# Aikku93/ulc-codec

Hardware: AMD Instinct MI355X
Metric: encode+decode Msamples/s at BlockSize=2048 stereo (channel-samples through encode+decode, VBR -50, 32 blocks per stream per call) (higher is better)
Workload: dtype f32; 1 GPU; vbr50 (configs[1] encode, configs[2] decode): Batch=4096 independent 44.1 kHz stereo streams/GPU x 32 blocks, BlockSize=2048, VBR -50; step = encode then decode; config=vbr50, mode=both, streams_per_gpu=4096, block_size=2048, channels=2, parallelism=batch split over 1 GPU(s), no collective on the data path

## Files before the change

ulc-codec_amd/csrc/ulcx_enc.hip:

```cpp
#include "ulcx_enc_dev.h"

static size_t ulcx_enc_xf_lds_bytes(int BS, int C) {
    if (BS > 8192) return (size_t)BS * 4;
    int ps = ulcx_xf_pad_shift(BS, C);
    size_t z = (size_t)4 * (BS + (BS >> ps)) * 4;
    size_t full = z + (size_t)BS * 2 + 32 + (C > 2 ? (size_t)BS * 2 : 0);
    return full <= ULCX_LDS_LIMIT ? full : z + (size_t)BS * 2 + 32;
}

static size_t ulcx_enc_xfa_lds_bytes(int BS, int C) {
    if (BS > 8192) return (size_t)BS * 4;
    int ps = ulcx_xf_pad_shift(BS, C);
    return (size_t)2 * (BS + (BS >> ps)) * 4 + (size_t)BS * 2 + 32;
}

#define CK(x) do { hipError_t e_ = (x); if (e_ != hipSuccess) { ulcx_set_error("%s: %s", #x, hipGetErrorString(e_)); return ULCX_ERR_HIP; } } while (0)
#define TRY(x) do { int rc_ = (x); if (rc_) return rc_; } while (0)

typedef void (*RangeKernel)(UlcxEncCtx, int, int);
typedef void (*PassKernel)(UlcxEncCtx, int);
typedef void (*CallKernel)(UlcxEncCtx);

static RangeKernel wc_energy_fn(const UlcxEncCtx &c) { return c.pcm16 ? k_wc_energy<int16_t> : k_wc_energy<float>; }
static RangeKernel wc_ef_fn(const UlcxEncCtx &c) { return c.pcm16 ? k_wc_ef<EF_NW, int16_t> : k_wc_ef<EF_NW, float>; }
static CallKernel state_update_fn(const UlcxEncCtx &c) { return c.pcm16 ? k_state_update<int16_t> : k_state_update<float>; }

template <typename IN> static RangeKernel xf_fn_in(const UlcxEncCtx &c, bool mdctOnly) {
    if (c.BS > 8192) return mdctOnly ? k_xfa_big<IN> : k_xf_big<IN>;
    if (c.C == 2) return mdctOnly ? k_xfa<true, IN> : k_xf<true, IN>;
    return mdctOnly ? k_xfa<false, IN> : k_xf<false, IN>;
}
static RangeKernel xf_fn(const UlcxEncCtx &c, bool mdctOnly) { return c.pcm16 ? xf_fn_in<int16_t>(c, mdctOnly) : xf_fn_in<float>(c, mdctOnly); }

template <int PASS> static PassKernel select_fn_pass(const UlcxEncCtx &c, bool pair, bool rates) {
#define SEL(R, L) (rates ? (PassKernel)k_select_wave_rates<R, L, PASS> : (PassKernel)k_select_wave<R, L, PASS>)
    switch (c.C * c.BS / 64) {
        case 128:
            if (pair) return rates ? k_select_pair_rates<64, 12, PASS> : k_select_pair<64, 12, PASS>;
            return SEL(128, 0);
        case 64: return c.lgBS == 11 ? SEL(64, 11) : SEL(64, 0);
        case 32: return SEL(32, 0);
        case 16: return SEL(16, 0);
        case 8:  return SEL(8, 0);
        case 4:  return SEL(4, 0);
        default: return nullptr;
    }
#undef SEL
}
static PassKernel select_fn(const UlcxEncCtx &c, bool pair, bool rates, int pass) {
    return pass == 1 ? select_fn_pass<1>(c, pair, rates) : pass == 2 ? select_fn_pass<2>(c, pair, rates) : select_fn_pass<0>(c, pair, rates);
}

static int allow_lds(const void *fn, size_t lds) {
    if (lds > 48 * 1024) CK(hipFuncSetAttribute(fn, hipFuncAttributeMaxDynamicSharedMemorySize, (int)lds));
    return ULCX_OK;
}

static void launch_wc_energy(const UlcxEncCtx &c, unsigned grid, hipStream_t st, int k0, int k1) {
    hipLaunchKernelGGL(wc_energy_fn(c), dim3(grid), dim3(WG), 0, st, c, k0, k1);
}

static void launch_wc_ef(const UlcxEncCtx &c, hipStream_t st, int k0, int k1) {
    static_assert(EF_LDS_BYTES <= 48 * 1024, "k_wc_ef: raise the dynamic LDS limit with hipFuncSetAttribute");
    hipLaunchKernelGGL(wc_ef_fn(c), dim3((c.B + EF_SPW - 1) / EF_SPW), dim3(EF_NW * 64), EF_LDS_BYTES, st, c, k0, k1);
}

static void launch_state_update(const UlcxEncCtx &c, hipStream_t st) {
    hipLaunchKernelGGL(state_update_fn(c), dim3(c.B), dim3(WG), 0, st, c);
}

const char *const ulcx_enc_stage_names[ULCX_ENC_STAGES_REPORTED] = {
    "k_wc_energy", "k_wc_forward", "k_wc_backward", "k_wc_integrate", "k_wc_decide",
    "k_xf", "k_cplx", "k_pbark", "k_mask",
    "k_select", "k_nbark", "(k_nline: gone)", "k_heapsel", "k_nsums", "k_tails", "k_encode_wave", "k_encode_units", "k_pack", "cbr_probe_passes", "k_state_update", "wc_pipeline_exposed",
};

struct StageMarks { hipEvent_t *ev; int stage; };
#define MARK(mk, s) do { if ((mk).ev) CK(hipEventRecord((mk).ev[(mk).stage++], s)); } while (0)

enum { ULCX_FRONT_ENCODE = 0, ULCX_FRONT_ANALYSE = 1, ULCX_FRONT_ANALYSE_KXF = 2, ULCX_FRONT_WC_ONLY = 3 };
static int launch_front(const UlcxEncCtx &c, hipStream_t st, StageMarks &mk, const UlcxEncAux &aux, const int what) {
    UlcxEncSync &sy = aux.sync;
    hipStream_t side = sy.side, side2 = sy.side2, side3 = sy.side3;
    const int SG = (c.B + 63) / 64;
    const int nCh = aux.wcPipe;
    const bool mdctOnly = (what == ULCX_FRONT_ANALYSE);
    const RangeKernel xf = (what == ULCX_FRONT_WC_ONLY) ? nullptr : xf_fn(c, mdctOnly);
    const size_t lds = mdctOnly ? ulcx_enc_xfa_lds_bytes(c.BS, c.C) : ulcx_enc_xf_lds_bytes(c.BS, c.C);
    if (xf) TRY(allow_lds((const void *)xf, lds));
    auto transform = [&](int k0, int k1) {
        if (xf) hipLaunchKernelGGL(xf, dim3((unsigned)((c.B * (k1 - k0) + 7) / 8) * 8), dim3(WG), lds, st, c, k0, k1);
    };
    const bool wcFuse = c.C == 2 && aux.wcFuse;
    aux.nXf = 0;
    if (nCh <= 1) {
        if (wcFuse) { MARK(mk, st); launch_wc_ef(c, st, 0, c.K);                                                  MARK(mk, st); }
        else {
        launch_wc_energy(c, (unsigned)(SG * ((c.K * c.BS) / 64)), st, 0, c.K);                                    MARK(mk, st);
        hipLaunchKernelGGL(k_wc_forward, dim3((c.B * 2 + 63) / 64), dim3(64), 0, st, c, 0, c.K);                  MARK(mk, st);
        }
        hipLaunchKernelGGL(k_wc_backward, dim3(SG * c.K), dim3(64), 0, st, c, 0, c.K);                            MARK(mk, st);
        hipLaunchKernelGGL(k_wc_integrate, dim3((c.B + 63) / 64), dim3(64), 0, st, c, 0, c.K);                    MARK(mk, st);
        hipLaunchKernelGGL(k_wc_decide, dim3((c.B * c.K + 63) / 64), dim3(64), 0, st, c, 0, c.K);                 MARK(mk, st);
        transform(0, c.K);
        MARK(mk, st);
        return ULCX_OK;
    }
    for (int i = 0; i < 5; i++) MARK(mk, st);
    int nW = aux.wcSteps;
    if (nW < 0) nW = (c.K >= 8) ? 4 : 0;
    if (nW > ULCX_WC_MAXCH) nW = ULCX_WC_MAXCH;
    if (nW > c.K) nW = c.K;
    const bool sameCuts = nW < 1;
    if (sameCuts) nW = nCh;
    int cut[ULCX_XF_MAXCH + 1];
    cut[0] = 0; cut[1] = 1;
    for (int j = 2; j <= nCh; j++) cut[j] = 1 + (c.K - 1) * (j - 1) / (nCh - 1);
    int wcs[ULCX_WC_MAXCH + 1];
    for (int w = 0; w <= nW; w++) wcs[w] = sameCuts ? cut[w] : (int)((long long)c.K * w / nW);
    CK(hipEventRecord(sy.wcStart, st));
    CK(hipStreamWaitEvent(side, sy.wcStart, 0));
    int jx = 0;
    for (int w = 0; w < nW; w++) {
        const int k0 = wcs[w], k1 = wcs[w + 1], kc = k1 - k0;
        if (wcFuse) launch_wc_ef(c, side, k0, k1);
        else {
            launch_wc_energy(c, (unsigned)(SG * ((kc * c.BS) / 64)), side, k0, k1);
            hipLaunchKernelGGL(k_wc_forward, dim3((c.B * 2 + 63) / 64), dim3(64), 0, side, c, k0, k1);
        }
        CK(hipEventRecord(sy.wcForward[w], side));
        CK(hipStreamWaitEvent(side2, sy.wcForward[w], 0));
        hipLaunchKernelGGL(k_wc_backward, dim3(SG * kc), dim3(64), 0, side2, c, k0, k1);
        CK(hipEventRecord(sy.wcBackward[w], side2));
        CK(hipStreamWaitEvent(side3, sy.wcBackward[w], 0));
        hipLaunchKernelGGL(k_wc_integrate, dim3((c.B + 63) / 64), dim3(64), 0, side3, c, k0, k1);
        hipLaunchKernelGGL(k_wc_decide, dim3((c.B * kc + 63) / 64), dim3(64), 0, side3, c, k0, k1);
        CK(hipEventRecord(sy.wcDecided[w], side3));
        while (jx < nCh && cut[jx + 1] <= k1) {
            CK(hipStreamWaitEvent(st, sy.wcDecided[w], 0));
            if (mk.ev) CK(hipEventRecord(sy.xfTiming[2 * jx], st));
            if (!(ULCX_DBG(c) & 0x2000))
            transform(cut[jx], cut[jx + 1]);
            if (mk.ev) CK(hipEventRecord(sy.xfTiming[2 * jx + 1], st));
            CK(hipEventRecord(sy.xfChunkDone[jx], st));
            jx++;
        }
    }
    aux.nXf = nCh;
    MARK(mk, st);
    for (int j = 0; j < nCh; j++) {
        CK(hipStreamWaitEvent(side, sy.xfChunkDone[j], 0));
        const int kc2 = cut[j + 1] - cut[j];
        if (what == ULCX_FRONT_ENCODE) hipLaunchKernelGGL(k_cplx, dim3((c.B * kc2 + 63) / 64), dim3(64), 0, side, c, cut[j], cut[j + 1]);
        else hipLaunchKernelGGL(k_cplxa, dim3((c.B * kc2 + 63) / 64), dim3(64), 0, side, c, cut[j], cut[j + 1]);
    }
    CK(hipEventRecord(sy.cplxChunksDone, side));
    return ULCX_OK;
}

struct EncPlan {
    int NB, N, nUnits;
    bool aside;
    int probes;
    size_t barkLds;
    bool selWave, selPair;
    size_t selLds;
    int ldsEntries, fbGrid; size_t heapLds;
    WaveCaps capS, capM, capF;
    bool haveFull, haveMid;
    int nsSlots;
};
static int enc_probes(const UlcxEncCtx &c, int N) {
    int n = 0;
    if (c.mode != ULCX_MODE_VBR || c.rates != nullptr) { n = 2; for (int m = N; m > 1; m >>= 1) n++; }
    return n;
}
static EncPlan enc_plan(const UlcxEncCtx &c, const UlcxEncAux &aux) {
    EncPlan p;
    p.NB = c.B * c.K; p.N = c.C * c.BS; p.nUnits = p.NB * c.C * 4;
    p.aside = aux.sync.side != nullptr;
    p.probes = enc_probes(c, p.N);
    p.barkLds = (size_t)c.barkRing * 3 * 64 * 8 + (size_t)2 * BK_TILE_FLOATS * 4;
    const int R = p.N / 64;
    p.selWave = (R == 4 || R == 8 || R == 16 || R == 32 || R == 64 || R == 128);
    p.selPair = (R == 128 && c.C == 2 && c.selPair);
    p.selLds = (size_t)(p.selPair ? 1 : 4) * ulcx_sel_lds_words(c.BS) * sizeof(float);
    p.ldsEntries = ((size_t)p.N * 8 <= ULCX_HEAP_LDS_BYTES) ? p.N : 0;
    p.heapLds = p.ldsEntries ? (size_t)p.N * 8 + (size_t)p.N / 8 : 0;
    p.fbGrid = p.NB < ULCX_HEAP_GRID ? p.NB : ULCX_HEAP_GRID;
    p.capS = { WAVE_SK, WAVE_SZ, WAVE_SN };
    p.capF = { (c.BS + 63) & ~63, ((c.BS / 2) + 63) & ~63, 4 * c.BS + 64 };
    while ((size_t)wavecaps_lds(p.capF) * 4 > 150 * 1024) {
        p.capF.k = (p.capF.k / 2 + 63) & ~63; p.capF.z = (p.capF.z / 2 + 63) & ~63; p.capF.nyb = p.capF.nyb / 2 + 32;
    }
    p.haveFull = p.capF.k > p.capS.k;
    p.capM = { 1024, 512, 4096 };
    p.haveMid = p.capM.k < p.capF.k;
    p.nsSlots = aux.nsSlots;
    return p;
}

static void launch_noise(const UlcxEncCtx &c, const EncPlan &p, hipStream_t s2) {
    if (c.barkRing) {
        hipLaunchKernelGGL(k_bark_uniform<true>, dim3((p.NB * c.C + 63) / 64), dim3(256), p.barkLds, s2, c);
        hipLaunchKernelGGL(k_bark_levels<true>, dim3((unsigned)(((size_t)p.NB * c.C * 32 + WG - 1) / WG)), dim3(WG), 0, s2, c);
    }
    hipLaunchKernelGGL(k_nbark, dim3((p.nUnits + 63) / 64), dim3(64), 0, s2, c, c.barkRing ? 1 : 0);
}

static int launch_psy(const UlcxEncCtx &c, const EncPlan &p, UlcxEncSync &sy, hipStream_t st, StageMarks &mk, bool cplxChunked) {
    if (c.barkRing) { TRY(allow_lds((const void *)k_bark_uniform<true>, p.barkLds)); TRY(allow_lds((const void *)k_bark_uniform<false>, p.barkLds)); }
    if (p.aside) {
        CK(hipEventRecord(sy.noiseFork, st));
        CK(hipStreamWaitEvent(sy.side3, sy.noiseFork, 0));
        if (cplxChunked) CK(hipStreamWaitEvent(sy.side3, sy.cplxChunksDone, 0));
        else hipLaunchKernelGGL(k_cplx, dim3((p.NB + 63) / 64), dim3(64), 0, sy.side3, c, 0, c.K);
        CK(hipEventRecord(sy.cplxDone, sy.side3));
        MARK(mk, st);
        launch_state_update(c, sy.side3);
        CK(hipEventRecord(sy.stateDone, sy.side3));
        CK(hipStreamWaitEvent(sy.side2, sy.noiseFork, 0));
        launch_noise(c, p, sy.side2);
        CK(hipEventRecord(sy.noiseDone, sy.side2));
    } else { hipLaunchKernelGGL(k_cplx, dim3((p.NB + 63) / 64), dim3(64), 0, st, c, 0, c.K);                MARK(mk, st); }
    const bool uniP = c.barkRing != 0;
    if (uniP) {
        hipLaunchKernelGGL(k_bark_uniform<false>, dim3((p.NB + 63) / 64), dim3(256), p.barkLds, st, c);
        hipLaunchKernelGGL(k_bark_levels<false>, dim3((unsigned)(((size_t)p.NB * 32 + WG - 1) / WG)), dim3(WG), 0, st, c);
    }
    hipLaunchKernelGGL(k_pbark, dim3((p.NB * 4 + 63) / 64), dim3(64), 0, st, c, uniP ? 1 : 0);            MARK(mk, st);
    MARK(mk, st);
    if (p.aside) CK(hipStreamWaitEvent(st, sy.cplxDone, 0));
    return ULCX_OK;
}

static int launch_select_wave(const UlcxEncCtx &c, const EncPlan &p, hipStream_t st, bool rates, int pass, int fin) {
    const PassKernel fn = select_fn(c, p.selPair, rates, pass);
    TRY(allow_lds((const void *)fn, p.selLds));
    if (p.selPair) hipLaunchKernelGGL(fn, dim3(p.NB), dim3(128), p.selLds, st, c, fin);
    else hipLaunchKernelGGL(fn, dim3((p.NB + 3) / 4), dim3(256), p.selLds, st, c, fin);
    return ULCX_OK;
}
static int launch_select(const UlcxEncCtx &c, const EncPlan &p, hipStream_t st, int fin) {
    if (!p.selWave) { hipLaunchKernelGGL(k_select, dim3(p.NB), dim3(WG), 0, st, c, fin); return ULCX_OK; }
    const bool rates = c.rates && c.selPass;
    TRY(launch_select_wave(c, p, st, rates, c.selPass, fin));
    if (rates && fin) TRY(launch_select_wave(c, p, st, true, 0, fin));
    return ULCX_OK;
}

static int launch_encode(const UlcxEncCtx &cc, const EncPlan &p, UlcxEncSync &sy, hipStream_t s2, int fin, StageMarks &mk) {
    const bool fb2 = (cc.fbMode == 2);
    const int NB = p.NB, fbW = NB < 128 ? NB : 128;
    if (cc.useGapSums) {
        const size_t glds = nsums_lds_bytes(p.N, cc.C);
        TRY(allow_lds((const void *)k_nsums, glds));
        const bool tailAside = !fb2 && p.aside;
        const unsigned tg = (unsigned)((p.nUnits + TAILS_U - 1) / TAILS_U);
        if (tailAside) {
            CK(hipEventRecord(sy.tailFork, s2));
            CK(hipStreamWaitEvent(sy.side2, sy.tailFork, 0));
            hipLaunchKernelGGL(k_tails, dim3(tg), dim3(WG), 0, sy.side2, cc, fin);
            CK(hipEventRecord(sy.tailDone, sy.side2));
        }
        const int nsGrid = NB < p.nsSlots ? NB : p.nsSlots;
        hipLaunchKernelGGL(k_nsums, dim3(fb2 ? fbW : nsGrid), dim3(WG), glds, s2, cc, fin);
        MARK(mk, s2);
        if (tailAside) CK(hipStreamWaitEvent(s2, sy.tailDone, 0));
        else hipLaunchKernelGGL(k_tails, dim3(fb2 ? fbW : tg), dim3(WG), 0, s2, cc, fin);
        MARK(mk, s2);
    } else { MARK(mk, s2); MARK(mk, s2); }
    if (cc.useWave) {
        const int nBC = NB * cc.C;
        hipLaunchKernelGGL(k_encode_wave<true>, dim3(fb2 ? fbW : (nBC + 3) / 4), dim3(256), (size_t)wavecaps_lds(p.capS) * 4 + 16, s2, cc, fin, p.capS, p.haveFull ? 0 : 2);
        if (p.haveFull) {
            const WaveCaps capR = (p.haveMid && (fb2 || (p.probes > 0 && !fin))) ? p.capM : p.capF;
            hipLaunchKernelGGL(k_encode_wave<false>, dim3(fb2 ? fbW : ((nBC + 3) / 4 < 512 ? (nBC + 3) / 4 : 512)), dim3(256), (size_t)wavecaps_lds(capR) * 4 + 16, s2, cc, fin, capR, 1);
        }
    }
    MARK(mk, s2);
    hipLaunchKernelGGL(k_encode_units, dim3(fb2 ? fbW : (p.nUnits + 63) / 64), dim3(64), 0, s2, cc, fin);
    MARK(mk, s2);
    if (!fin && !fb2) hipLaunchKernelGGL(k_rate_step, dim3((NB + 255) / 256), dim3(256), 0, s2, cc);
    else hipLaunchKernelGGL(k_pack, dim3(fb2 ? (fbW + 3) / 4 : (NB + 3) / 4), dim3(256), 0, s2, cc, fin);
    MARK(mk, s2);
    return ULCX_OK;
}

static UlcxEncCtx exact_ctx(const UlcxEncCtx &c, int lo) { UlcxEncCtx cf = c; cf.fbMode = 2; cf.fbLo = lo; cf.fbHi = lo + c.rankSlots; return cf; }
static void exact_sort(const UlcxEncCtx &c, const EncPlan &p, hipStream_t s2, int lo) {
    const UlcxEncCtx cf = exact_ctx(c, lo);
    if (p.ldsEntries) hipLaunchKernelGGL(k_heapsel_pipe, dim3(p.fbGrid), dim3(64), p.heapLds, s2, cf, p.probes > 0 ? 1 : 0);
    else hipLaunchKernelGGL(k_heapsel, dim3(p.fbGrid), dim3(64), p.heapLds, s2, cf, p.ldsEntries);
}
static int exact_passes(const UlcxEncCtx &c, const EncPlan &p, UlcxEncSync &sy, hipStream_t s2, int lo) {
    const UlcxEncCtx cf = exact_ctx(c, lo);
    StageMarks none = { nullptr, 0 };
    for (int pass = 0; pass <= p.probes; pass++) {
        const int fin = (pass == p.probes) ? 1 : 0;
        const bool fromSort = (p.probes == 0 && p.ldsEntries);
        if (!fromSort) hipLaunchKernelGGL(k_keep_ranks, dim3(p.fbGrid), dim3(WG), 0, s2, cf, fin);
        if (cf.useWave && !(fromSort && lo == 0)) CK(hipMemsetAsync(cf.slow + p.NB + 1, 0, sizeof(int), s2));
        TRY(launch_encode(cf, p, sy, s2, fin, none));
    }
    return ULCX_OK;
}

static int launch_passes(UlcxEncCtx &c, const EncPlan &p, UlcxEncSync &sy, hipStream_t st, StageMarks &mk, bool first) {
    const int NB = p.NB;
    StageMarks none = { nullptr, 0 };
    for (int pass = 0; pass <= p.probes; pass++) {
        const int fin = (pass == p.probes) ? 1 : 0;
        StageMarks &m = (pass == 0) ? mk : none;
        const bool async_fb = p.aside && fin;
        if (c.useWave && pass > 0) CK(hipMemsetAsync(c.slow, 0, sizeof(int) * ((size_t)NB + 2), st));
        c.selPass = (p.probes > 0 && !c.keyFinal) ? (pass == 0 ? 1 : 2) : 0;
        TRY(launch_select(c, p, st, fin));
        MARK(m, st);
        if (async_fb) {
            CK(hipEventRecord(sy.exactFork, st));
            CK(hipStreamWaitEvent(sy.side, sy.exactFork, 0));
            exact_sort(c, p, sy.side, 0);
        }
        if (pass == 0) {
            if (first) {
                if (p.aside) CK(hipStreamWaitEvent(st, sy.noiseDone, 0));
                else launch_noise(c, p, st);
            }
            MARK(m, st); MARK(m, st);
        }
        if (async_fb) {
            CK(hipEventRecord(sy.exactFork2, st));
            CK(hipStreamWaitEvent(sy.side, sy.exactFork2, 0));
            TRY(exact_passes(c, p, sy, sy.side, 0));
            for (int lo = c.rankSlots; lo < NB; lo += c.rankSlots) {
                exact_sort(c, p, sy.side, lo);
                TRY(exact_passes(c, p, sy, sy.side, lo));
            }
            CK(hipEventRecord(sy.exactJoin, sy.side));
        }
        MARK(m, st);
        UlcxEncCtx cm = c; cm.fbMode = 1;
        TRY(launch_encode(cm, p, sy, st, fin, m));
        if (async_fb) CK(hipStreamWaitEvent(st, sy.exactJoin, 0));
    }
    if (!p.aside) {
        for (int lo = 0; lo < NB; lo += c.rankSlots) {
            exact_sort(c, p, st, lo);
            TRY(exact_passes(c, p, sy, st, lo));
        }
    }
    return ULCX_OK;
}

int ulcx_enc_launch_ladder(const UlcxEncCtx *rungs, int nRungs, hipStream_t st, hipEvent_t *ev, const UlcxEncAux &aux) {
    UlcxEncCtx c = rungs[0];
    UlcxEncSync &sy = aux.sync;
    const EncPlan p = enc_plan(c, aux);
    StageMarks mk = { ev, 0 }, none = { nullptr, 0 };
    if (p.probes) CK(hipMemsetAsync(c.cbrLive, 0, sizeof(int), st));
    if (c.barkRing) CK(hipMemsetAsync(c.decCount, 0, sizeof(int), st));
    if (nRungs > 1) CK(hipMemsetAsync(c.fbCount + 1, 0, sizeof(int), st));
    MARK(mk, st);
    TRY(launch_front(c, st, mk, aux, ULCX_FRONT_ENCODE));
    if (ULCX_DBG(c) & 0x6000) { MARK(mk, st); return ULCX_OK; }
    TRY(launch_psy(c, p, sy, st, mk, aux.wcPipe > 1));
    if (!p.selWave) { ulcx_enc_finalize_keys(c, st); c.keyFinal = 1; }
    TRY(allow_lds((const void *)k_heapsel, p.heapLds)); TRY(allow_lds((const void *)k_heapsel_pipe, p.heapLds));
    if (p.haveFull && (size_t)wavecaps_lds(p.capF) * 4 > 48 * 1024) CK(hipFuncSetAttribute((const void *)k_encode_wave<false>, hipFuncAttributeMaxDynamicSharedMemorySize, wavecaps_lds(p.capF) * 4 + 16));
    TRY(launch_passes(c, p, sy, st, mk, true));
    for (int r = 1; r < nRungs; r++) {
        UlcxEncCtx cr = rungs[r];
        cr.keyFinal = c.keyFinal;
        EncPlan pr = p;
        pr.probes = enc_probes(cr, p.N);
        if (pr.probes) CK(hipMemsetAsync(cr.cbrLive, 0, sizeof(int), st));
        ulcx_enc_rung_arm(cr, st);
        TRY(launch_passes(cr, pr, sy, st, none, false));
    }
    MARK(mk, st);
    if (p.aside) CK(hipStreamWaitEvent(st, sy.stateDone, 0));
    else launch_state_update(c, st);
    MARK(mk, st);
    CK(hipGetLastError());
    return ULCX_OK;
}

int ulcx_enc_launch(const UlcxEncCtx &c, hipStream_t st, hipEvent_t *ev, const UlcxEncAux &aux) {
    return ulcx_enc_launch_ladder(&c, 1, st, ev, aux);
}

int ulcx_analyse_launch(const UlcxEncCtx &c, hipStream_t st, hipEvent_t *ev, const UlcxEncAux &aux, int useKxf) {
    const int what = !c.cplxOut ? ULCX_FRONT_WC_ONLY : useKxf ? ULCX_FRONT_ANALYSE_KXF : ULCX_FRONT_ANALYSE;
    if (what == ULCX_FRONT_ANALYSE_KXF && c.barkRing) CK(hipMemsetAsync(c.decCount, 0, sizeof(int), st));
    StageMarks mk = { ev, 0 };
    MARK(mk, st);
    TRY(launch_front(c, st, mk, aux, what));
    if (aux.wcPipe > 1) CK(hipStreamWaitEvent(st, aux.sync.cplxChunksDone, 0));
    else hipLaunchKernelGGL(k_cplxa, dim3((c.B * c.K + 63) / 64), dim3(64), 0, st, c, 0, c.K);
    MARK(mk, st);
    while (mk.ev && mk.stage < ULCX_ENC_STAGES) MARK(mk, st);
    launch_state_update(c, st);
    MARK(mk, st);
    CK(hipGetLastError());
    return ULCX_OK;
}
```

ulc-codec_amd/csrc/ulcx_enc_wr.hip:

```cpp
#include "ulcx_enc_dev.h"

__device__ __forceinline__ float run_amplitude(const float *pairs, int start, int n) {
    const float2 *d = (const float2 *)(pairs + (start / 2) * 2);
    const int np = (n + (start & 1) + 1) / 2;
    float sum = 0.0f, sumw = 0.0f;
    int q = 0;
    for (; q + 8 <= np; q += 8) {
        float2 p[8];
#pragma unroll
        for (int u = 0; u < 8; u++) p[u] = d[q + u];
#pragma unroll
        for (int u = 0; u < 8; u++) { sum += p[u].y; sumw += p[u].x; }
    }
    for (; q < np; q++) { float2 p = d[q]; sum += p.y; sumw += p.x; }
    return (sum == 0.0f) ? -1.0f : ulcx_expf(sum / sumw);
}

#define NS_KW 2

#define NS_BK 7

struct NsPre { uint32_t kw[NS_KW]; float bk[NS_BK]; int wc; };

__device__ __forceinline__ void nsums_fetch(const UlcxEncCtx &c, int blk, NsPre &p) {
// ... 511 lines not shown
            const int iw = __builtin_amdgcn_ds_bpermute(lo << 2, incl);
            int r = jj - (iw - __popc(ww));
            uint32_t t = ww; int pos = 0;
#pragma unroll
            for (int sh = 16; sh >= 1; sh >>= 1) {
                const int cl = __popc(t & ((1u << sh) - 1u));
                const bool up = r >= cl;
                r = up ? r - cl : r; t = up ? t >> sh : t; pos = up ? pos + sh : pos;
            }
            const int idx = (wb + lo) * 32 + pos;
            if (pendAt >= 0) kval[pendAt] = pendV;
            const bool mine = j < tot && nK + j < E2_KCAP;
            pendAt = mine ? nK + j : -1;
            if (mine) { kidx[nK + j] = (uint16_t)idx; pendV = coefU[idx]; }
        }
        nK += tot;
    }
    if (pendAt >= 0) kval[pendAt] = pendV;
    bool overflow = nK > E2_KCAP;
    WAVE_SYNC();
    if ((ULCX_DBG(c) >> 8) == 1) { if (lane == 0) c.unitNyb[gid] = 0; return; }

    int nZ = 0;
    if (!overflow && nK > 0) {
        const uint32_t INFB = 0x7F800000u;
        uint32_t cmn = 0u, cmx = 0u;
        bool open = false;
        for (int base = 0; base < nK; base += 64) {
            const int i = base + lane;
            const uint32_t lv = (i < nK) ? (__float_as_uint(kval[i]) & 0x7FFFFFFFu) : INFB;
            int myz = 0;
            int s = 0;
            for (;;) {
                uint32_t a = lv;
                if (base == 0 && s == 0 && lane == 0) a = (__uint_as_float(lv) < 1000.0f) ? lv : __float_as_uint(1000.0f);
                a = (lane >= s) ? a : 0xFFFFFFFFu;
                uint32_t b = (lane >= s) ? lv : 0u;
#define STEP(ctl, rmask) { uint32_t o = (uint32_t)__builtin_amdgcn_update_dpp((int)0xFFFFFFFFu, (int)a, ctl, rmask, 0xf, false); a = o < a ? o : a; \
                           uint32_t q = (uint32_t)__builtin_amdgcn_update_dpp(0, (int)b, ctl, rmask, 0xf, false); b = q > b ? q : b; }
                ULCX_DPP_STEPS(STEP)
#undef STEP
                if (open) { a = cmn < a ? cmn : a; b = cmx > b ? cmx : b; }
                const bool brk = (__uint_as_float(b) > __uint_as_float(a) * 4.0f) && (open || lane > s);
                const unsigned long long m = __ballot(brk);
                if (m == 0ull) {
                    if (lane >= s) myz = nZ;
                    cmn = (uint32_t)__builtin_amdgcn_readlane((int)a, 63); cmx = (uint32_t)__builtin_amdgcn_readlane((int)b, 63);
                    open = true;
                    break;
                }
                const int t = __builtin_ctzll(m);
                if (lane >= s && lane < t) myz = nZ;
                const uint32_t zm = t > 0 ? (uint32_t)__builtin_amdgcn_readlane((int)b, t - 1) : cmx;
                if (lane == 0 && nZ < E2_ZCAP) ((uint32_t *)zmax)[nZ] = zm;
                nZ++;
                s = t; open = false;
                if (base + t >= nK) break;
            }
            if (i < nK) kz[i] = (uint16_t)myz;
        }
        if (open) { if (lane == 0 && nZ < E2_ZCAP) ((uint32_t *)zmax)[nZ] = cmx; nZ++; }
        WAVE_SYNC();
        if (nZ <= E2_ZCAP && __builtin_amdgcn_readfirstlane((int)((uint32_t *)zmax)[nZ - 1]) == 0) nZ--;
        if (nZ > E2_ZCAP) overflow = true;
    }
    WAVE_SYNC();
    if ((ULCX_DBG(c) >> 8) == 2) { if (lane == 0) c.unitNyb[gid] = 0; return; }

    if (!overflow) {
        int run = 0;
        for (int base = 0; base < nZ; base += 64) {
            int z = base + lane;
            int qn = 0;
            if (z < nZ) { int qi = build_quantizer(zmax[z]); zqi[z] = (int8_t)qi; }
            WAVE_SYNC();
            if (z < nZ) {
                int qi = zqi[z];
                int prev = (z > 0) ? zqi[z - 1] : -1;
                if (qi != prev) qn = ((z > 0) ? 1 : 0) + ((qi - 5 < 0xE) ? 1 : 2);
            }
            int tot, ex = wave_excl_scan(qn, lane, tot);
            if (z < nZ) zpre[z] = run + ex + qn;
            run += tot;
        }
    }
    WAVE_SYNC();
    if ((ULCX_DBG(c) >> 8) == 3) { if (lane == 0) c.unitNyb[gid] = 0; return; }

    int nC = 0;
    if (!overflow) {
        bool prevCodedCarry = true;
        for (int base = 0; base < nK; base += 64) {
            int kk = base + lane;
            bool coded = false; int qn = 0, idx = 0, z = 0;
            if (kk < nK) {
                z = kz[kk]; idx = kidx[kk];
                float cq = kval[kk] * (float)(1u << zqi[z]);
                coded = !(fabsf(cq) < 2.5f);
                qn = quant_coef(cq, 7);
            }
            unsigned long long m = __ballot(coded);
            unsigned long long valid = __ballot(kk < nK);
            bool prevCoded = (lane == 0) ? prevCodedCarry : (((m >> (lane - 1)) & 1) != 0);
            int pos = nC + __popcll(m & ((1ull << lane) - 1));
            if (coded) { kidx[pos] = (uint16_t)(idx | (prevCoded ? 0x8000 : 0)); kz[pos] = (uint16_t)z; ((int *)kval)[pos] = qn; }
            int lastValid = 63 - __clzll(valid);
            prevCodedCarry = ((m >> lastValid) & 1) != 0;
            nC += __popcll(m);
        }
    }
    WAVE_SYNC();
    if ((ULCX_DBG(c) >> 8) == 4) { if (lane == 0) c.unitNyb[gid] = 0; return; }

    int total = 0;
    if (!overflow) {
        auto gap_amps = [&](int m) {
            float2 a = make_float2(-2.0f, -2.0f);
            if (m < nC) {
                const int raw = kidx[m], idx = raw & 0x7FFF, start = (m > 0) ? (kidx[m - 1] & 0x7FFF) + 1 : 0;
                if (idx - start >= 16 && (raw & 0x8000) && c.useGapSums) a = gapU[idx];
            }
            return a;
        };
        float2 ampR = gap_amps(lane);
        for (int base = 0; base < nC; base += 64) {
            int m = base + lane;
            unsigned long long lo = 0, hi = 0; int cnt = 0, pre = 0, z = 0, zp = -1, qn = 0;
            const float2 ampN = gap_amps(m + 64);
            if (m < nC) {
                int raw = kidx[m];
                int idx = raw & 0x7FFF;
                int start = (m > 0) ? (kidx[m - 1] & 0x7FFF) + 1 : 0;
                z = kz[m]; zp = (m > 0) ? kz[m - 1] : -1;
                qn = ((int *)kval)[m];
                pre = zpre[z] - ((zp >= 0) ? zpre[zp] : 0);
                int zr = idx - start;
                const float amp0 = ampR.x, amp1 = ampR.y;
                gap_codes(start, zr, (float)(1u << zqi[z]), coefU, src, ubase, amp0, amp1, amp0 > -1.5f ? gapU + idx : nullptr, lo, hi, cnt, (ULCX_DBG(c) & 0x40) != 0);
            }
            int mine = (m < nC) ? pre + cnt + 1 : 0;
            int tot, ex = wave_excl_scan(mine, lane, tot);
            if (cnt > 32) overflow = true;
            int p = total + ex;
            if (m < nC && finalPass && p + mine <= E2_NYBCAP && cnt <= 32) {
                for (int zz = zp + 1; zz <= z; zz++) {
                    int qi = zqi[zz], prev = (zz > 0) ? zqi[zz - 1] : -1;
                    if (qi != prev) {
                        if (zz > 0) nyb[p++] = 0xF;
                        int sft = qi - 5;
                        if (sft < 0xE) nyb[p++] = (uint8_t)sft; else { nyb[p++] = 0xE; nyb[p++] = (uint8_t)(sft - 0xE); }
                    }
                }
                for (int q = 0; q < cnt; q++) nyb[p++] = (uint8_t)(((q < 16) ? (lo >> (4 * q)) : (hi >> (4 * (q - 16)))) & 0xF);
                nyb[p++] = (uint8_t)(qn & 0xF);
            }
            total += tot;
            ampR = ampN;
        }
        overflow = __any(overflow);
    }
    if ((ULCX_DBG(c) >> 8) == 5) { if (lane == 0) c.unitNyb[gid] = 0; return; }

    if (!overflow) {
        int zlast = (nC > 0) ? kz[nC - 1] : -1;
        int nextCoded = (nC > 0) ? (kidx[nC - 1] & 0x7FFF) + 1 : 0;
        int n = S - nextCoded;
        int prevQ = (nZ > 0) ? zqi[nZ - 1] : -1;
        int qtail = ((nZ > 0) ? zpre[nZ - 1] : 0) - ((zlast >= 0) ? zpre[zlast] : 0);
        int nq = 0, nd = 0;
        if (n > 4 && prevQ != -1 && n >= 16) {
            float sx, sx2, sxy, sy, sw;
            if (c.useGapSums && __float_as_int(tsB.y) == ubase + nextCoded) {
                sx = tsA.x; sx2 = tsA.y; sxy = tsA.z; sy = tsA.w; sw = tsB.x;
            } else {
                const int p0 = (ubase + nextCoded) / 2;
                int np = (n + (nextCoded & 1) + 1) / 2;
                float acc = 0.0f;
                if (lane < 5) {
                    for (int i = 0; i < np; i++) {
                        float2 pv = pair_demand(src, p0 + i);
                        float x = i * 2.0f;
                        float wx = pv.x * x;
                        float term = (lane == 0) ? wx : (lane == 1) ? wx * x : (lane == 2) ? x * pv.y : (lane == 3) ? pv.y : pv.x;
                        acc += term;
                    }
                }
                sx = __shfl(acc, 0); sx2 = __shfl(acc, 1); sxy = __shfl(acc, 2); sy = __shfl(acc, 3); sw = __shfl(acc, 4);
            }
            hfext_from_sums(sx, sx2, sxy, sy, sw, (float)(1u << prevQ), nq, nd);
        }
        int tailN = 0;
        if (n > 4) tailN = ((prevQ != -1) ? 1 : 0) + (nq ? 4 : 2);
        else if (n > 0) tailN = 2;
        int p = total + qtail;
        if (finalPass && lane == 0 && p + tailN <= E2_NYBCAP) {
            int q0 = total;
            for (int zz = zlast + 1; zz < nZ; zz++) {
                int qi = zqi[zz], prev = (zz > 0) ? zqi[zz - 1] : -1;
                if (qi != prev) {
                    if (zz > 0) nyb[q0++] = 0xF;
                    int sft = qi - 5;
                    if (sft < 0xE) nyb[q0++] = (uint8_t)sft; else { nyb[q0++] = 0xE; nyb[q0++] = (uint8_t)(sft - 0xE); }
                }
            }
            if (n > 4) {
                if (prevQ != -1) nyb[p++] = 0xF;
                if (nq) { nyb[p++] = 0xF; nyb[p++] = (uint8_t)(nq - 1); nyb[p++] = (uint8_t)((nd >> 4) & 0xF); nyb[p++] = (uint8_t)(nd & 0xF); }
                else { nyb[p++] = 0xE; nyb[p++] = 0xF; }
            } else if (n > 0) { nyb[p++] = 0x0; nyb[p++] = (uint8_t)(n - 1); }
        }
        total += qtail + tailN;
        if (total > E2_NYBCAP) overflow = true;
    }
    const bool direct = xch != nullptr;
    if (overflow) {
        if (direct && ch == 0 && lane == 0) __hip_atomic_store(xch, XCH_WORD(0, 0, 1, seq), __ATOMIC_RELAXED, __HIP_MEMORY_SCOPE_WORKGROUP);
        if (lane == 0) {
            int old = atomicOr(&c.slow[blk], failBit);
            if (failBit == 1 && !(old & 1)) {
                const int NBq = c.B * c.K, which = (c.fbMode == 2) ? 1 : 0;
                int q = atomicAdd(&c.slow[NBq + which], 1);
                c.slow[NBq + 2 + which * NBq + q] = blk;
            }
        }
        return;
    }
    WAVE_SYNC();
    if (lane == 0) c.unitNyb[gid] = total;
    if (!finalPass) return;
    if (direct) {
        int o = 1; uint32_t prevNyb = (uint32_t)wc & 0xFu;
        bool ok = true;
        if (ch == 0) {
            if (lane == 0) __hip_atomic_store(xch, XCH_WORD(total, total ? nyb[total - 1] : prevNyb, 0, seq), __ATOMIC_RELAXED, __HIP_MEMORY_SCOPE_WORKGROUP);
        } else {
            unsigned long long v64;
            for (;;) {
                v64 = __hip_atomic_load(xch, __ATOMIC_RELAXED, __HIP_MEMORY_SCOPE_WORKGROUP);
                if ((uint32_t)(v64 >> 32) == (uint32_t)seq) break;
                __builtin_amdgcn_s_sleep(2);
            }
            const uint32_t v = (uint32_t)__builtin_amdgcn_readfirstlane((int)(uint32_t)v64);
            ok = !((v >> 20) & 1u);
            o = 1 + (int)(v & 0xFFFFu); prevNyb = (v >> 16) & 0xFu;
        }
        if (ok) {
            const int end = o + total;
            const int bEnd = ch == 0 ? end >> 1 : (end + 1) >> 1;
            uint8_t *outB = c.out + (size_t)blk * c.slot;
            for (int b = (o >> 1) + lane; b < bEnd; b += 64) {
                const int q0 = 2 * b - o;
                const unsigned lo4 = q0 >= 0 ? nyb[q0] : prevNyb;
                const unsigned hi4 = q0 + 1 < total ? nyb[q0 + 1] : 0u;
                if (b < c.slot) outB[b] = (uint8_t)(lo4 | (hi4 << 4));
            }
            if (ch == 1 && lane == 0) { c.bits[blk] = (end * 4 + 7) & ~7; atomicOr(&c.slow[blk], 4); }
            return;
        }
    }
    uint8_t *dst = c.unitBuf + (size_t)blk * c.C * c.unitCap + (size_t)ch * c.unitCap + 2 * off + 8 * j;
    int nb = (total + 1) / 2;
    for (int b = lane; b < nb; b += 64) {
        unsigned lo4 = nyb[2 * b];
        unsigned hi4 = (2 * b + 1 < total) ? nyb[2 * b + 1] : 0;
        dst[b] = (uint8_t)(lo4 | (hi4 << 4));
    }
}

template <bool SMALL>
__global__ __launch_bounds__(256, SMALL ? EW_LB : 1) void k_encode_wave(UlcxEncCtx c, int finalPass, WaveCaps caps, int phase) {
    if (probes_over(c, finalPass)) return;
    extern __shared__ float e2all[];
    const int wv = __builtin_amdgcn_readfirstlane(threadIdx.x >> 6), lane = threadIdx.x & 63;
    const WaveCaps capS = { WAVE_SK, WAVE_SZ, WAVE_SN };
    const int ldsPerWave = SMALL ? wavecaps_lds(capS) : wavecaps_lds(caps);
    float *e2 = (float *)((char *)e2all + (size_t)wv * ldsPerWave);
    const int NBq = c.B * c.K, which = (c.fbMode == 2) ? 1 : 0;
    const int *queue = c.slow + NBq + 2 + which * NBq;
    int nBlk = (phase == 1) ? c.slow[NBq + which] : (c.fbMode == 2) ? fb_count(c) : NBq;
    unsigned long long *xchAll = (unsigned long long *)((char *)e2all + 4 * (size_t)ldsPerWave);
    const bool directOK = finalPass && c.C == 2 && phase != 1 && c.directPack && (long long)gridDim.x * 4 >= (long long)nBlk * c.C;
    if (directOK) { if (threadIdx.x < 2) xchAll[threadIdx.x] = 0; __syncthreads(); }
    int seq = 0;
    for (int u = blockIdx.x * 4 + wv; u < nBlk * c.C; u += gridDim.x * 4) {
        seq++;
        int blk = u / c.C, ch = u - blk * c.C;
        if (phase == 1) blk = queue[blk];
        else {
            if (c.fbMode == 2) blk = c.fbList[c.fbLo + blk];
            if (skip_block(c, blk, finalPass)) continue;
        }
        int s = blk / c.K, k = blk % c.K;
        const int nW0 = c.BS >> 5;
        const uint32_t kwPre = (lane < nW0) ? c.keep[(size_t)blk * (c.C * c.BS / 32) + (size_t)ch * nW0 + lane] : 0u;
        int wc = c.wcArr[(size_t)s * (c.maxK + 2) + k + 1];
        const bool whole = (c.BS >> (ulcx_pattern(wc) & 7)) == c.BS;
        for (int j = 0; j < 4; j++) {
            encode_unit_wave<SMALL>(c, finalPass, blk, ch, j, wc, lane, e2, caps, phase ? 2 : 1, (directOK && whole && j == 0) ? xchAll + (wv >> 1) : nullptr, seq, kwPre, j == 0);
            WAVE_SYNC();
        }
    }
}

__device__ void pack_block(const UlcxEncCtx &c, int finalPass, int blk) {
    int lane = threadIdx.x & 63;
    if (skip_block(c, blk, finalPass)) return;
    if (finalPass && c.useWave && (c.slow[blk] & 4)) return;
    int s = blk / c.K, k = blk % c.K;
    int wc = c.wcArr[(size_t)s * (c.maxK + 2) + k + 1];
    int nU = c.C * 4;
    const int *un = c.unitNyb + (size_t)blk * nU;
    int hdr = (wc & 8) ? 2 : 1;
    int total = hdr;
    for (int u = 0; u < nU; u++) total += un[u];
    int bitsTot = ((total * 4) + 7) & ~7;
    if (!finalPass) {
        if (lane == 0) {
            int budget = c.cbrBudget[blk];
            int lo = c.cbrLo[blk], hi = c.cbrHi[blk], nOut = c.nout[blk];
            bool stop = false;
            if (bitsTot < budget) lo = nOut;
            else if (bitsTot > budget) hi = nOut - 1;
            else { lo = nOut; stop = true; }
            if (stop || !(lo < hi - 1)) { c.cbrDone[blk] = 1; c.nout[blk] = lo; if (c.fbMode != 2) atomicSub(c.cbrLive, 1); }
            else c.nout[blk] = (int)((unsigned)(lo + hi) / 2u);
            c.cbrLo[blk] = lo; c.cbrHi[blk] = hi;
            if (c.selPass && c.fbMode != 2 && nOut > 0) {
                const uint32_t T = c.selT[blk];
                uint4 w = c.selWin[blk];
                if (bitsTot > budget) { w.x = T; w.z = (uint32_t)nOut; }
                else { w.y = T; w.w = (uint32_t)nOut; }
                c.selWin[blk] = w;
            }
        }
        return;
    }
    uint8_t *out = c.out + (size_t)blk * c.slot;
    int nBytes = bitsTot / 8;
    const uint8_t *ub = c.unitBuf + (size_t)blk * c.C * c.unitCap;
    for (int b = lane; b < nBytes; b += 64) {
        unsigned byte = 0;
        for (int h = 0; h < 2; h++) {
            int q = 2 * b + h;
            unsigned nyb = 0;
            if (q < hdr) nyb = (q == 0) ? (wc & 0xF) : ((wc >> 4) & 0xF);
            else if (q < total) {
                int r = q - hdr;
                int u = 0;
                while (r >= un[u]) { r -= un[u]; u++; }
                int ch = u >> 2, j = u & 3;
                int d, off, S;
                unit_geom(wc, j, c.BS, d, off, S);
                const uint8_t *src = ub + (size_t)ch * c.unitCap + 2 * off + 8 * j;
                nyb = (src[r >> 1] >> ((r & 1) * 4)) & 0xF;
            }
            byte |= nyb << (4 * h);
        }
        if (b < c.slot) out[b] = (uint8_t)byte;
    }
    if (lane == 0) c.bits[blk] = bitsTot;
}

__global__ __launch_bounds__(256) void k_rate_step(UlcxEncCtx c) {
    if (probes_over(c, 0)) return;
    const int blk = blockIdx.x * 256 + threadIdx.x;
    bool ended = false;
    if (blk < c.B * c.K && !skip_block(c, blk, 0)) {
        const int s = blk / c.K, k = blk % c.K;
        const int wc = c.wcArr[(size_t)s * (c.maxK + 2) + k + 1];
        const int nU = c.C * 4;
        const int *un = c.unitNyb + (size_t)blk * nU;
        int total = (wc & 8) ? 2 : 1;
        for (int u = 0; u < nU; u++) total += un[u];
        const int bitsTot = ((total * 4) + 7) & ~7;
        const int budget = c.cbrBudget[blk];
        int lo = c.cbrLo[blk], hi = c.cbrHi[blk];
        const int nOut = c.nout[blk];
        bool stop = false;
        if (bitsTot < budget) lo = nOut;
        else if (bitsTot > budget) hi = nOut - 1;
        else { lo = nOut; stop = true; }
        if (stop || !(lo < hi - 1)) { c.cbrDone[blk] = 1; c.nout[blk] = lo; ended = true; }
        else c.nout[blk] = (int)((unsigned)(lo + hi) / 2u);
        c.cbrLo[blk] = lo; c.cbrHi[blk] = hi;
        if (c.selPass && nOut > 0) {
            const uint32_t T = c.selT[blk];
            uint4 w = c.selWin[blk];
            if (bitsTot > budget) { w.x = T; w.z = (uint32_t)nOut; }
            else { w.y = T; w.w = (uint32_t)nOut; }
            c.selWin[blk] = w;
        }
    }
    const unsigned long long e = __ballot(ended);
    if (e && (threadIdx.x & 63) == 0) atomicSub(c.cbrLive, (int)__popcll(e));
}

__global__ __launch_bounds__(256) void k_pack(UlcxEncCtx c, int finalPass) {
    if (probes_over(c, finalPass)) return;
    const int wv = threadIdx.x >> 6;
    if (c.fbMode != 2) { const int blk = blockIdx.x * 4 + wv; if (blk < c.B * c.K) pack_block(c, finalPass, blk); return; }
    int n = fb_count(c);
    for (int v = blockIdx.x * 4 + wv; v < n; v += gridDim.x * 4) pack_block(c, finalPass, c.fbList[c.fbLo + v]);
}

int ulcx_enc_nsums_slots(int BS, int C) {
    const size_t lds = nsums_lds_bytes(C * BS, C);
    if (lds > 48 * 1024 && hipFuncSetAttribute((const void *)k_nsums, hipFuncAttributeMaxDynamicSharedMemorySize, (int)lds) != hipSuccess) { (void)hipGetLastError(); return 0; }
    int dev = 0, cus = 0, per = 0;
    if (hipGetDevice(&dev) != hipSuccess || hipDeviceGetAttribute(&cus, hipDeviceAttributeMultiprocessorCount, dev) != hipSuccess) { (void)hipGetLastError(); return 0; }
    if (hipOccupancyMaxActiveBlocksPerMultiprocessor(&per, (const void *)k_nsums, WG, lds) != hipSuccess) { (void)hipGetLastError(); return 0; }
    return cus * per;
}

template __global__ void k_encode_wave<false>(UlcxEncCtx, int, WaveCaps, int);
template __global__ void k_encode_wave<true>(UlcxEncCtx, int, WaveCaps, int);
```

ulc-codec_amd/csrc/ulcx_internal.h:

```cpp
#pragma once
#include <hip/hip_runtime.h>
#include <stdint.h>
#include "../../include/ulc_amd.h"

#ifndef ULCX_DSYN_TWL
#define ULCX_DSYN_TWL 1
#endif
#define ULCX_NBARK 25
#define ULCX_MAX_SUB 4
#define ULCX_BARK_EVENTS 52
#define ULCX_MAX_BS_DEVICE 32768
#define ULCX_COEF_EPS (0x1.0p-31f)
#define ULCX_HEAP_LDS_BYTES (128 * 1024)
#define ULCX_HEAP_GRID 256
#define ULCX_DONE_VBR 2
#ifdef ULCX_ABLATE
#define ULCX_DBG(c) ((c).dbgSkip)
#else
#define ULCX_DBG(c) 0
#endif

struct UlcxTables {
    const float2 *pre[ULCX_MAX_SUB];
    const float2 *tw[ULCX_MAX_SUB];
    const float  *winFall;
    const float  *winRise;
    const int    *bandIdx[ULCX_MAX_SUB];
    const float  *bandFrac[ULCX_MAX_SUB];
    const float4 *bandW[ULCX_MAX_SUB];
    const uint32_t *barkSched;
    short nBeg[ULCX_MAX_SUB][ULCX_NBARK], nEnd[ULCX_MAX_SUB][ULCX_NBARK];
    short pBeg[ULCX_MAX_SUB][ULCX_NBARK], pEnd[ULCX_MAX_SUB][ULCX_NBARK];
};

struct UlcxWcState {
    float tf[3];
    int   wcPrev, wcCur;
    float binSum[8], binW[8];
    int   pad;
};

struct UlcxEncCtx {
    int B, K, C, BS, lgBS;
    int barkRing;
    int *decList, *decCount;
    int maxK;
    int slot;
    int unitCap;
    int mode; float p0, p1;
    float vbrTarget;
    const float2 *rates;
    float cHP, cBP, qHP, qBP, cBlk;
    float cplxScale;
    int   rateHz;
    UlcxTables T;
    int keyFinal;
    const float *pcm; const int16_t *pcm16;
    uint8_t *out; int32_t *bits; int32_t *wcOut; float *cplxOut;
    float *hist;
    UlcxWcState *wcs;
    float2 *env;
    float  *bins;
    int    *wcArr;
    float  *coef;
    float  *key;
    float  *nsum;
    float  *npair;
    float  *amp2;
    float  *barkN;
    float  *barkP;
    double *barkRawN, *barkRawP;
    int    *nnz;
    float  *cplx;
    int    *nout;
    int    *cbrLo, *cbrHi, *cbrDone;
    uint32_t *keep;
    int    *fbList; int *fbCount;
    uint8_t *unitBuf;
    int    *unitNyb;
    int    *cbrBudget;
    uint4  *selWin;
    uint32_t *selT;
    int     selPair;
    int     selPass;
    int    *cbrLive;
    int    *slow;
    float2 *gapSum;
    float  *tailSum;
    int     useGapSums;
    int    *isFb;
    int    *ownSlot;
    int    *rankBuf;
    int     dbgSkip;
    int     forceFb;
    int     rankSlots, fbLo, fbHi;
    int     fbMode;
    int     useWave;
    int     directPack;
    void   *heapScratch;
};

struct UlcxDecCtx {
    int B, K, C, BS, lgBS, maxK;
    int s0, s1;
    int slot;
    int dbgSkip;
    UlcxTables T;
    const uint8_t *in; float *pcm; int16_t *pcm16;
    long long inBytes;
    int32_t *bits;
    float *lap;
    int   *lastSub;
    uint32_t *seed;
    int   *dead;
    float *lapO; int *lastSubO; uint32_t *seedO; int *deadO;
    float *lapScratch;
    int    synFull;
    int    k0, k1;
    int   *wcScan;
    int   *draws;
    int   *unitDraws;
    float4 *unitTail;
    int4  *unitRec;
    uint2 *prec; int precStride;
    uint2 *nrec; int nrecStride;
    float *tailMag;
    int    tailStride;
    float *scratch;
    const uint32_t *jumpT;
    const uint32_t *parT;
    int    fastOK, twInLds;
    int   packed;
    long long payStride;
    const int32_t *payBytes;
    int  *packOff;
    int  *blkOff;
    int   range;
    const ulcx_index_entry *rIndex;
    int   rIndexStride;
    const int32_t *rIndexBlocks, *rFirst;
    int2 *rInfo;
    int32_t *bitsOut;
};

__host__ __device__ static inline unsigned ulcx_pattern(int wc) {
    const unsigned i = ((unsigned)wc >> 4) & 15u;
    const unsigned long long t0 = 0x0091001900080000ull, t1 = 0x0A2102A101A2012Aull, t2 = 0x1B3213B212B3123Bull, t3 = 0xB3213B212B3123B1ull;
    const unsigned long long t = (i & 8u) ? ((i & 4u) ? t3 : t2) : ((i & 4u) ? t1 : t0);
    return (unsigned)(t >> (16u * (i & 3u))) & 0xFFFFu;
}

int  ulcx_tables_build(UlcxTables *devT, void **devBlob, int BS, int rateHz, bool forEncoder);
void ulcx_set_error(const char *fmt, ...);

#define ULCX_ENC_STAGES 20
#define ULCX_ENC_STAGES_REPORTED (ULCX_ENC_STAGES + 1)
extern const char *const ulcx_enc_stage_names[ULCX_ENC_STAGES_REPORTED];
#define ULCX_DEC_STAGES 2
#define ULCX_WC_MAXCH 32
#define ULCX_XF_MAXCH 8
#define ULCX_LDS_LIMIT (160 * 1024)
struct UlcxEncSync {
    hipEvent_t wcStart, wcForward[ULCX_WC_MAXCH], wcBackward[ULCX_WC_MAXCH], wcDecided[ULCX_WC_MAXCH];
    hipEvent_t xfChunkDone[ULCX_XF_MAXCH], cplxChunksDone;
    hipEvent_t noiseFork, noiseDone, tailFork, tailDone;
    hipEvent_t cplxDone, stateDone;
    hipEvent_t exactFork, exactFork2, exactJoin;
    hipEvent_t xfTiming[2 * ULCX_XF_MAXCH];
    hipStream_t side, side2, side3;
};
struct UlcxEncAux {
    UlcxEncSync &sync;
    int wcPipe;
    int wcSteps, wcFuse, nsSlots;
    int &nXf;
};
int ulcx_enc_launch(const UlcxEncCtx &c, hipStream_t st, hipEvent_t *ev , const UlcxEncAux &aux);
int ulcx_enc_launch_ladder(const UlcxEncCtx *rungs, int nRungs, hipStream_t st, hipEvent_t *ev, const UlcxEncAux &aux);
void ulcx_enc_rung_arm(const UlcxEncCtx &c, hipStream_t st);
struct UlcxDecAux {
    int synGrid;
    int synFull;
};
int ulcx_dec_launch(const UlcxDecCtx &c, hipStream_t st, hipEvent_t *ev, const UlcxDecAux &aux);
int ulcx_index_launch(const UlcxDecCtx &c, int maxBlocks, ulcx_index_entry *d_index, int32_t *d_nBlocks, hipStream_t st);
size_t ulcx_dec_lds_bytes(int BS, int fast, int twInLds);
int ulcx_dec_syn_slots(const UlcxDecCtx &c);
int ulcx_pack_launch(int nStreams, int nBlocks, int slotBytes, const uint8_t *d_slots, const int32_t *d_bits, uint8_t *d_payload,
                     long long stride, int32_t *d_payloadBytes, int32_t *d_maxBlock, hipStream_t st);
int ulcx_analyse_launch(const UlcxEncCtx &c, hipStream_t st, hipEvent_t *ev, const UlcxEncAux &aux, int useKxf);
int ulcx_enc_nsums_slots(int BS, int C);
__host__ __device__ static inline int ulcx_xf_pad_shift(int BS, int C) { (void)BS; (void)C; return 4; }
#define ULCX_SEL_CAP 8
#ifndef ULCX_SEL_CAND
#define ULCX_SEL_CAND 128
#endif
__host__ __device__ static inline int ulcx_sel_lds_words(int BS) { int a = BS / 2 + 4 * ULCX_NBARK, b = ULCX_SEL_CAP * 64; return a > b ? a : b; }
struct UlcxSlotRows {
    uint8_t *hdr; size_t hdrStride;
    uint8_t *big; size_t bigStride;
    uint8_t *small[4]; size_t smallStride;
};
struct UlcxSlotGeom {
    int B;
    int rowVec;
    int isEnc, nSmall, smallWords;
    int padWords;
    uint4 header;
};
int ulcx_slots_gather(const UlcxSlotRows &obj, const UlcxSlotRows &rows, const int32_t *d_slots, int n, const UlcxSlotGeom &g, hipStream_t st);
int ulcx_slots_scatter(const UlcxSlotRows &obj, const UlcxSlotRows &rows, const int32_t *d_slots, int n, const UlcxSlotGeom &g, hipStream_t st);
int ulcx_slots_reset(const UlcxSlotRows &obj, const int32_t *d_slots, int n, const UlcxSlotGeom &g, hipStream_t st);
void ulcx_enc_finalize_keys(const UlcxEncCtx &c, hipStream_t st);
void ulcx_enc_materialise_noise(const UlcxEncCtx &c, hipStream_t st);
```

Measured before the change: 56050 Msamples/s.

## Overlap pbark on side stream, skip wave retry in fallback, word-pack output

When the side stream is enabled, k_pbark now launches on side3 ahead of k_cplx, and the main stream waits on a new pbarkDone event. This lets it overlap with the bark-uniform and level kernels. The second encode_wave retry pass is dropped in fallback mode (fb2). pack_block now assembles 32-bit words from unit runs, with unrolled prefix sizes and unaligned 64-bit reads, instead of extracting nibble by nibble through a per-nibble unit search. These changes add a new event, which must be created somewhere not shown here, and the new packing is more intricate and carries bit-exactness risk.

Result: slower. 55280 Msamples/s (-1.4%).

```diff
diff --git a/ulc-codec_amd/csrc/ulcx_enc.hip b/ulc-codec_amd/csrc/ulcx_enc.hip
--- a/ulc-codec_amd/csrc/ulcx_enc.hip
+++ b/ulc-codec_amd/csrc/ulcx_enc.hip
@@ -210,9 +210,13 @@
 
 static int launch_psy(const UlcxEncCtx &c, const EncPlan &p, UlcxEncSync &sy, hipStream_t st, StageMarks &mk, bool cplxChunked) {
     if (c.barkRing) { TRY(allow_lds((const void *)k_bark_uniform<true>, p.barkLds)); TRY(allow_lds((const void *)k_bark_uniform<false>, p.barkLds)); }
+    const bool uniP = c.barkRing != 0;
+    auto pbark = [&](hipStream_t s) { hipLaunchKernelGGL(k_pbark, dim3((p.NB * 4 + 63) / 64), dim3(64), 0, s, c, uniP ? 1 : 0); };
     if (p.aside) {
         CK(hipEventRecord(sy.noiseFork, st));
         CK(hipStreamWaitEvent(sy.side3, sy.noiseFork, 0));
+        pbark(sy.side3);
+        CK(hipEventRecord(sy.pbarkDone, sy.side3));
         if (cplxChunked) CK(hipStreamWaitEvent(sy.side3, sy.cplxChunksDone, 0));
         else hipLaunchKernelGGL(k_cplx, dim3((p.NB + 63) / 64), dim3(64), 0, sy.side3, c, 0, c.K);
         CK(hipEventRecord(sy.cplxDone, sy.side3));
@@ -223,14 +227,14 @@
         launch_noise(c, p, sy.side2);
         CK(hipEventRecord(sy.noiseDone, sy.side2));
     } else { hipLaunchKernelGGL(k_cplx, dim3((p.NB + 63) / 64), dim3(64), 0, st, c, 0, c.K);                MARK(mk, st); }
-    const bool uniP = c.barkRing != 0;
     if (uniP) {
         hipLaunchKernelGGL(k_bark_uniform<false>, dim3((p.NB + 63) / 64), dim3(256), p.barkLds, st, c);
         hipLaunchKernelGGL(k_bark_levels<false>, dim3((unsigned)(((size_t)p.NB * 32 + WG - 1) / WG)), dim3(WG), 0, st, c);
     }
-    hipLaunchKernelGGL(k_pbark, dim3((p.NB * 4 + 63) / 64), dim3(64), 0, st, c, uniP ? 1 : 0);            MARK(mk, st);
-    MARK(mk, st);
-    if (p.aside) CK(hipStreamWaitEvent(st, sy.cplxDone, 0));
+    if (!p.aside) pbark(st);
+    MARK(mk, st);
+    MARK(mk, st);
+    if (p.aside) { CK(hipStreamWaitEvent(st, sy.cplxDone, 0)); CK(hipStreamWaitEvent(st, sy.pbarkDone, 0)); }
     return ULCX_OK;
 }
 
@@ -272,10 +276,11 @@
     } else { MARK(mk, s2); MARK(mk, s2); }
     if (cc.useWave) {
         const int nBC = NB * cc.C;
-        hipLaunchKernelGGL(k_encode_wave<true>, dim3(fb2 ? fbW : (nBC + 3) / 4), dim3(256), (size_t)wavecaps_lds(p.capS) * 4 + 16, s2, cc, fin, p.capS, p.haveFull ? 0 : 2);
-        if (p.haveFull) {
-            const WaveCaps capR = (p.haveMid && (fb2 || (p.probes > 0 && !fin))) ? p.capM : p.capF;
-            hipLaunchKernelGGL(k_encode_wave<false>, dim3(fb2 ? fbW : ((nBC + 3) / 4 < 512 ? (nBC + 3) / 4 : 512)), dim3(256), (size_t)wavecaps_lds(capR) * 4 + 16, s2, cc, fin, capR, 1);
+        const bool retry = p.haveFull && !fb2;
+        hipLaunchKernelGGL(k_encode_wave<true>, dim3(fb2 ? fbW : (nBC + 3) / 4), dim3(256), (size_t)wavecaps_lds(p.capS) * 4 + 16, s2, cc, fin, p.capS, retry ? 0 : 2);
+        if (retry) {
+            const WaveCaps capR = (p.haveMid && p.probes > 0 && !fin) ? p.capM : p.capF;
+            hipLaunchKernelGGL(k_encode_wave<false>, dim3((nBC + 3) / 4 < 512 ? (nBC + 3) / 4 : 512), dim3(256), (size_t)wavecaps_lds(capR) * 4 + 16, s2, cc, fin, capR, 1);
         }
     }
     MARK(mk, s2);
diff --git a/ulc-codec_amd/csrc/ulcx_enc_wr.hip b/ulc-codec_amd/csrc/ulcx_enc_wr.hip
--- a/ulc-codec_amd/csrc/ulcx_enc_wr.hip
+++ b/ulc-codec_amd/csrc/ulcx_enc_wr.hip
@@ -837,6 +837,14 @@
     }
 }
 
+__device__ __forceinline__ int pack_unit_size(int u, int s0, int s1, int s2, int s3, int s4, int s5, int s6, int s7, const int *un) {
+    int v = s0;
+    v = (u == 1) ? s1 : v; v = (u == 2) ? s2 : v; v = (u == 3) ? s3 : v; v = (u == 4) ? s4 : v;
+    v = (u == 5) ? s5 : v; v = (u == 6) ? s6 : v; v = (u == 7) ? s7 : v;
+    if (u >= 8) v = un[u];
+    return v;
+}
+
 __device__ void pack_block(const UlcxEncCtx &c, int finalPass, int blk) {
     int lane = threadIdx.x & 63;
     if (skip_block(c, blk, finalPass)) return;
@@ -872,27 +880,46 @@
     }
     uint8_t *out = c.out + (size_t)blk * c.slot;
     int nBytes = bitsTot / 8;
-    const uint8_t *ub = c.unitBuf + (size_t)blk * c.C * c.unitCap;
-    for (int b = lane; b < nBytes; b += 64) {
-        unsigned byte = 0;
-        for (int h = 0; h < 2; h++) {
-            int q = 2 * b + h;
-            unsigned nyb = 0;
-            if (q < hdr) nyb = (q == 0) ? (wc & 0xF) : ((wc >> 4) & 0xF);
-            else if (q < total) {
-                int r = q - hdr;
-                int u = 0;
-                while (r >= un[u]) { r -= un[u]; u++; }
-                int ch = u >> 2, j = u & 3;
+    const int s0 = un[0], s1 = un[1], s2 = un[2], s3 = un[3];
+    const int s4 = nU > 4 ? un[4] : 0, s5 = nU > 4 ? un[5] : 0, s6 = nU > 4 ? un[6] : 0, s7 = nU > 4 ? un[7] : 0;
+#define PACK_SIZE_OF(u) pack_unit_size(u, s0, s1, s2, s3, s4, s5, s6, s7, un)
+    const uint32_t *ub32 = (const uint32_t *)c.unitBuf;
+    const size_t ubOff = (size_t)blk * c.C * c.unitCap;
+    const int lim = nBytes < c.slot ? nBytes : c.slot;
+    const bool outAligned = ((uintptr_t)out & 3) == 0;
+    for (int w = lane; 4 * w < lim; w += 64) {
+        const int q0 = 8 * w;
+        uint32_t word = 0;
+        if (w == 0) word = (hdr == 2) ? (wc & 0xFF) : (wc & 0xF);
+        int q = q0 < hdr ? hdr : q0;
+        const int qe = (q0 + 8 < total) ? q0 + 8 : total;
+        int r = q - hdr, u = 0;
+        bool on = true;
+#pragma unroll
+        for (int i = 0; i < 8; i++) { const int si = PACK_SIZE_OF(i); on = on && i < nU && r >= si; if (on) { r -= si; u++; } }
+        while (u >= 8 && u < nU && r >= un[u]) { r -= un[u]; u++; }
+        while (q < qe && u < nU) {
+            const int left = PACK_SIZE_OF(u) - r;
+            if (left > 0) {
+                const int n = (qe - q < left) ? qe - q : left;
+                const int ch = u >> 2, j = u & 3;
                 int d, off, S;
                 unit_geom(wc, j, c.BS, d, off, S);
-                const uint8_t *src = ub + (size_t)ch * c.unitCap + 2 * off + 8 * j;
-                nyb = (src[r >> 1] >> ((r & 1) * 4)) & 0xF;
-            }
-            byte |= nyb << (4 * h);
-        }
-        if (b < c.slot) out[b] = (uint8_t)byte;
-    }
+                const size_t row = ubOff + (size_t)ch * c.unitCap + 2 * off + 8 * j;
+                const size_t o = row + (r >> 1), oLast = row + ((r + left - 1) >> 1);
+                const size_t i0 = o >> 2, i1 = (i0 + 1 < (oLast >> 2)) ? i0 + 1 : (oLast >> 2);
+                const uint64_t two = (uint64_t)ub32[i0] | ((uint64_t)ub32[i1] << 32);
+                const uint32_t bits = (uint32_t)(two >> (((int)(o & 3)) * 8 + (r & 1) * 4));
+                const uint32_t mask = (n == 8) ? 0xFFFFFFFFu : ((1u << (4 * n)) - 1u);
+                word |= (bits & mask) << (4 * (q - q0));
+                q += n;
+            }
+            u++; r = 0;
+        }
+        if (outAligned && 4 * w + 4 <= lim) *(uint32_t *)(out + 4 * w) = word;
+        else for (int b = 4 * w; b < lim && b < 4 * w + 4; b++) out[b] = (uint8_t)(word >> (8 * (b - 4 * w)));
+    }
+#undef PACK_SIZE_OF
     if (lane == 0) c.bits[blk] = bitsTot;
 }
 
diff --git a/ulc-codec_amd/csrc/ulcx_internal.h b/ulc-codec_amd/csrc/ulcx_internal.h
--- a/ulc-codec_amd/csrc/ulcx_internal.h
+++ b/ulc-codec_amd/csrc/ulcx_internal.h
@@ -165,6 +165,7 @@
     hipEvent_t xfChunkDone[ULCX_XF_MAXCH], cplxChunksDone;
     hipEvent_t noiseFork, noiseDone, tailFork, tailDone;
     hipEvent_t cplxDone, stateDone;
+    hipEvent_t pbarkDone;
     hipEvent_t exactFork, exactFork2, exactJoin;
     hipEvent_t xfTiming[2 * ULCX_XF_MAXCH];
     hipStream_t side, side2, side3;
```
